# laurentsenta/testground

Measured on AMD Instinct MI355X. Metric: simulated packets/sec (whole node) at 10k & 1M peers; % of HBM roofline, higher is better.
Workload: dtype u32/u64 integer

## Files before the change

testground_amd/build.py:

```python
from __future__ import annotations

import os
import subprocess
from pathlib import Path

PKG = Path(__file__).resolve().parent
ROOT = PKG.parent
CSRC = PKG / "csrc"
LIB = PKG / "libtgsim.so"
SOURCES = [CSRC / "tgsim_kernels.hip", CSRC / "tgsim_engine.cpp", CSRC / "tgsim_bridge.cpp", CSRC / "tgsim_comm.cpp"]
HEADERS = [CSRC / "tgsim_internal.h", CSRC / "tgsim_launch.h", ROOT / "include" / "tgsim.h"]
ORACLE_DIR = ROOT / "oracle"
ORACLE_LIB = ORACLE_DIR / "build" / "libtgoracle.so"

HIPCC = os.environ.get("HIPCC", "/opt/rocm/bin/hipcc")
ARCH = os.environ.get("PYTORCH_ROCM_ARCH", "gfx950")


def _stale(target: Path, deps) -> bool:
    if not target.exists():
        return True
    t = target.stat().st_mtime
    return any(Path(d).stat().st_mtime > t for d in deps)


PROF_LIB = PKG / "libtgsim_prof.so"
CHECK_LIB = PKG / "libtgsim_check.so"


def build_engine(force: bool = False, verbose: bool = False, profile: bool = False, check: bool = False) -> Path:
    lib = PROF_LIB if profile else CHECK_LIB if check else LIB
    if not force and not _stale(lib, SOURCES + HEADERS):
        return lib
    objs = []
    build_dir = PKG / ("build_prof" if profile else "build_check" if check else "build")
    build_dir.mkdir(exist_ok=True)
    for src in SOURCES:
        obj = build_dir / (src.stem + ".o")
        dev = ["-mllvm", "-amdgpu-use-amdgpu-trackers=1", "-mllvm", "-disable-promote-alloca-to-lds"] \
            if src.suffix == ".hip" else []
        cmd = [HIPCC, f"--offload-arch={ARCH}", "-O3", "-std=c++17", "-fPIC", "-Wall", *dev,
               "-Wno-unused-result", *(["-DTGSIM_PROFILE"] if profile else []),
               *(["-DTGSIM_CHECK"] if check else []), "-c", str(src), "-o", str(obj)]
        if verbose:
            print(" ".join(cmd))
        subprocess.run(cmd, check=True)
        objs.append(str(obj))
    cmd = [HIPCC, f"--offload-arch={ARCH}", "-shared", "-fPIC", "-o", str(lib), *objs]
    if verbose:
        print(" ".join(cmd))
    subprocess.run(cmd, check=True)
    return lib


def build_oracle(force: bool = False) -> Path:
    if os.environ.get("TGORACLE_LIB"):
        return Path(os.environ["TGORACLE_LIB"])
    if force or _stale(ORACLE_LIB, [ORACLE_DIR / "tgoracle.c", ORACLE_DIR / "tgoracle.h", ROOT / "include" / "tgsim.h"]):
        subprocess.run(["make", "-C", str(ORACLE_DIR), "-B" if force else "all"], check=True,
                       stdout=subprocess.DEVNULL)
    return ORACLE_LIB


MOCK_DIR = ROOT / "tests" / "mockrccl"
# ... 37 lines not shown
```

testground_amd/csrc/tgsim_internal.h:

```cpp
#pragma once
#include <hip/hip_runtime.h>
#include <stdint.h>

#include "../../include/tgsim.h"

namespace tgsim {

constexpr uint32_t kHeapCap = 1024;
constexpr uint32_t kWave = 64;
#ifndef TGSIM_SPW
#define TGSIM_SPW 1
#endif
constexpr uint32_t kSpw = TGSIM_SPW;
constexpr uint32_t kAhead = kWave / kSpw;
constexpr uint64_t kEMask = (1ull << 46) - 1;
constexpr uint32_t kStates = TGSIM_SYNC_STATES;
constexpr uint32_t kDeadDst = 0xFFFFFFFFu;

struct alignas(16) SrcParams {
  uint64_t lat_ns;
  uint64_t burst_ns;
  int32_t sigma;
  uint32_t mult;
  uint32_t shift_ext;
// ... 49 lines not shown
  uint32_t last_dup, last_cor, last_reo, _pad;
  SrcParams p;
};

enum StatSlot {
  kStOffered = 0, kStScheduled, kStCloned, kStCorrupted, kStVerdict0,
  kStBytes = 12, kStErr = 13, kStQueue = 14, kStLost = 15, kStFlushed = 16,
  kStCarrySkip = 17,
  kStBktRecs = 18,
  kStSlots = 20
};
#ifndef TGSIM_STAT_COPIES
#define TGSIM_STAT_COPIES 2048
#endif
constexpr uint32_t kStatCopies = TGSIM_STAT_COPIES;
constexpr uint32_t kErrTimeOverflow = 1u;

struct SimArgs {
  const SrcParams* params;
  SrcState* state;
  const uint8_t* enabled;
  const uint32_t* ip;
  const Interval* rules;
  const uint64_t* off;
  const InRec* in;
  uint8_t* verdict;
  uint4* heap;
  uint64_t* ring;
  tgsim_delivery* emit;
  uint32_t* emit_n;
  unsigned long long* stats;
  uint32_t key0, key1;
  uint32_t n_src, shard_begin, n_peers, queue_limit;
  uint32_t any_disabled;
  uint64_t t0_ns, tick_ns, horizon_ns;
  const uint32_t* order;
  uint64_t* stamps;
  unsigned long long* dst_cnt;
  uint64_t* err_host;
  uint32_t* worklist;
  tgsim_delivery* emit_pool;
  uint32_t* emit_pool_idx;
  uint32_t* g_first;
  uint64_t* g_pend;
  const uint64_t* g_fwd;
  uint32_t g_floods, g_degree;
  tgsim_delivery* dst_bkt;
  uint32_t emit_r : 24, bkt_log : 7, dst_slot : 1;
  uint32_t emit_pool_cap;
  uint4* wheel;
  WheelMeta* wmeta;
};
static_assert(sizeof(SimArgs) == 280, "SimArgs layout");
constexpr uint32_t kStampSlots = 32;

constexpr uint32_t kFuseMax = 8;
struct FusedWindow {
  const uint64_t* off;
  const InRec* in;
  uint8_t* verdict;
  tgsim_delivery* emit;
  uint32_t* emit_n;
  unsigned long long* dst_cnt;
  uint64_t t0_ns, horizon_ns;
};
struct FusedArgs {
  FusedWindow w[kFuseMax];
  uint32_t n_win;
  uint32_t step_base;
  uint32_t ticket_base;
  uint32_t* ticket;
  uint32_t* done;
  uint32_t prio_n;
  uint32_t persistent;
};
constexpr uint32_t kErrHandoff = 2u;
constexpr uint32_t kErrDeliverCap = 4u;
constexpr uint32_t kErrEmitPool = 8u;

struct EmitRead {
  const tgsim_delivery* base;
  const tgsim_delivery* pool;
  const uint32_t* pool_idx;
  uint32_t r;
  uint32_t slot;
  const tgsim_delivery* bkt;
  uint32_t bkt_log, _pad;
  const uint64_t* guard_total;
  uint64_t guard_cap;
};
constexpr uint32_t kSlotShift = 46;
constexpr uint32_t kBktLogMin = 3, kBktLogMax = 6;
#if defined(TGSIM_CHECK) && !defined(TGSIM_CHECK_FULL_SLOTS)
constexpr uint64_t kSlotNone = (1u << kBktLogMax) + 3;
#else
constexpr uint64_t kSlotNone = (1ull << (64 - kSlotShift)) - 1;
#endif
static_assert(kSlotNone >= (1u << kBktLogMax), "the fallback places records behind every bucket slot");
__host__ __device__ inline uint64_t slot_bits(unsigned long long rank) {
  return (uint64_t)(rank < kSlotNone ? rank : kSlotNone) << kSlotShift;
}
__host__ __device__ inline const tgsim_delivery* emit_rec(const EmitRead& e, uint32_t s, uint64_t o0, uint64_t o1,
                                                         uint32_t i, uint32_t pidx) {
  const uint64_t cap = 2 * (o1 - o0) + e.r;
  return i < cap ? e.base + 2 * o0 + (uint64_t)e.r * s + i : e.pool + pidx + (i - cap);
}
struct GroupDeliver {
// ... 50 lines not shown
```

testground_amd/csrc/tgsim_kernels.hip:

```cpp
#include <errno.h>
#include <stdlib.h>
#include "tgsim_launch.h"

namespace tgsim {

__device__ __forceinline__ void philox(uint32_t c0, uint32_t c1, uint32_t c2, uint32_t c3,
                                       uint32_t k0, uint32_t k1, uint32_t r[4]) {
  __asm__ volatile("" : "+s"(k0), "+s"(k1));
#pragma unroll
  for (int i = 0; i < 10; ++i) {
    const uint64_t p0 = (uint64_t)0xD2511F53u * c0, p1 = (uint64_t)0xCD9E8D57u * c2;
    const uint32_t h0 = (uint32_t)(p0 >> 32), l0 = (uint32_t)p0;
    const uint32_t h1 = (uint32_t)(p1 >> 32), l1 = (uint32_t)p1;
    const uint32_t n0 = h1 ^ c1 ^ k0, n2 = h0 ^ c3 ^ k1;
    c0 = n0; c1 = l1; c2 = n2; c3 = l0;
    k0 += 0x9E3779B9u;
    k1 += 0xBB67AE85u;
  }
  r[0] = c0; r[1] = c1; r[2] = c2; r[3] = c3;
}

__device__ __forceinline__ uint32_t crand(uint32_t raw, uint32_t rho, uint32_t& last) {
  if (rho == 0) return raw;
  const uint64_t r = (uint64_t)rho + 1;
  const uint32_t a = (uint32_t)(((uint64_t)raw * ((1ull << 32) - r) + (uint64_t)last * r) >> 32);
  last = a;
  return a;
}

__device__ __forceinline__ uint64_t w0_of(const uint4& a) {
  return ((uint64_t)a.y << 32) | a.x;
}
__device__ __forceinline__ bool item_lt(const uint4& a, const uint4& b) {
  const uint64_t ea = w0_of(a) & kEMask, eb = w0_of(b) & kEMask;
  const bool dup_first = (a.y >> 30 & 1u) > (b.y >> 30 & 1u);
  const bool seq_lt = (a.z < b.z) | ((a.z == b.z) & dup_first);
  return (ea < eb) | ((ea == eb) & seq_lt);
}

template <uint32_t kCap>
struct SimLdsT {
  uint4 slot[kCap];
  uint32_t wcnt[kWheelB];
  uint32_t whdr[4];
};
static_assert(sizeof(SimLdsT<kHeapCap>) <= 65536, "simulate workgroup LDS");

constexpr uint32_t kFvPass = 0xFFu;

#ifdef TGSIM_CHECK
__device__ unsigned int tg_exec_faults;
__device__ unsigned int tg_exec_lines[8192];
__device__ __noinline__ void tg_exec_fault(const char* what, uint64_t exec, uint32_t l, int line) {
  const uint32_t me = __lane_id();
// ... 64 lines not shown
__device__ __forceinline__ void scan_maxplus(uint64_t& a, uint64_t& b, int line = __builtin_LINE()) {
#define STEP(C, R) { const uint64_t pa = dpp64<C, R>(0, a, line), pb = dpp64<C, R>(0, b, line); \
                     const uint64_t nb = pb + a; b = nb > b ? nb : b; a = pa + a; }
  TG_SCAN_STEPS(STEP)
#undef STEP
}
__device__ __forceinline__ int32_t scan_sum_i32(int32_t v, int line = __builtin_LINE()) {
#define STEP(C, R) v += (int32_t)dpp<C, R>(0u, (uint32_t)v, line);
  TG_SCAN_STEPS(STEP)
#undef STEP
  return v;
}
__device__ __forceinline__ int32_t scan_max_i32(int32_t v, int line = __builtin_LINE()) {
#define STEP(C, R) v = max(v, (int32_t)dpp<C, R>(0x80000000u, (uint32_t)v, line));
  TG_SCAN_STEPS(STEP)
#undef STEP
  return v;
}
__device__ __forceinline__ uint32_t scan_max_u32(uint32_t v, int line = __builtin_LINE()) {
#define STEP(C, R) v = max(v, dpp<C, R>(0u, v, line));
  TG_SCAN_STEPS(STEP)
#undef STEP
  return v;
}
__device__ __forceinline__ uint64_t scan_max_u64(uint64_t v, int line = __builtin_LINE()) {
#define STEP(C, R) { const uint64_t p = dpp64<C, R>(0ull, v, line); v = p > v ? p : v; }
  TG_SCAN_STEPS(STEP)
#undef STEP
  return v;
}
__device__ __forceinline__ uint64_t scan_min_u64(uint64_t v, int line = __builtin_LINE()) {
#define STEP(C, R) { const uint64_t p = dpp64<C, R>(~0ull, v, line); v = p < v ? p : v; }
  TG_SCAN_STEPS(STEP)
#undef STEP
  return v;
}

__device__ __forceinline__ uint32_t count_le_sorted_u32(uint32_t v, uint32_t t, int line = __builtin_LINE()) {
  TG_FULL_EXEC_AT("count_le_sorted", line);
  uint32_t lo = 0;
#pragma unroll
  for (uint32_t s = 32; s; s >>= 1)
    if ((uint32_t)__shfl(v, (int)(lo + s - 1), 64) <= t) lo += s;
  return lo + ((uint32_t)__shfl(v, (int)lo, 64) <= t ? 1u : 0u);
}

__device__ __forceinline__ uint64_t delayed(const SrcParams& p, uint64_t T, uint32_t raw) {
  if (p.sigma == 0) return T + p.lat_ns;
  const uint32_t m = 2u * (uint32_t)p.sigma;
  const int64_t delay = (int64_t)(raw % m) + (int64_t)p.lat_ns - (int64_t)p.sigma;
  return delay > 0 ? T + (uint64_t)delay : T;
}

struct RecvFold {
  uint32_t* first;
  uint64_t* pend;
  const uint64_t* fwd;
  uint32_t floods, degree, shard_begin, n_local;
  uint64_t tick_ns;
  double inv_tick;
};
__device__ __forceinline__ RecvFold recv_fold(const SimArgs& a) {
  return RecvFold{a.g_first, a.g_pend,  a.g_fwd,   a.g_floods,
                  a.g_degree, a.shard_begin, a.n_src, a.tick_ns, 1.0 / (double)a.tick_ns};
}
__device__ __forceinline__ void fold_receipt(const RecvFold& g, uint32_t dst, uint32_t seq, uint32_t flags, uint64_t d,
                                             uint64_t fw) {
  const uint32_t f = seq / g.degree, s = dst - g.shard_begin;
  if (s >= g.n_local || f >= g.floods || (flags & TGSIM_FLAG_CORRUPT) || (fw >> f & 1ull)) return;
  uint64_t q = (uint64_t)((double)d * g.inv_tick);
  const int64_t r = (int64_t)(d - q * g.tick_ns);
  q = r < 0 ? q - 1 : (uint64_t)r >= g.tick_ns ? q + 1 : q;
  uint64_t t = q + 1;
  if (t > 0xFFFFFFFEull) t = 0xFFFFFFFEull;
  if (__hip_atomic_fetch_min(&g.first[(uint64_t)s * 64 + f], (uint32_t)t, __ATOMIC_RELAXED, __HIP_MEMORY_SCOPE_AGENT) ==
      0xFFFFFFFFu)
    __hip_atomic_fetch_or(&g.pend[s], 1ull << f, __ATOMIC_RELAXED, __HIP_MEMORY_SCOPE_AGENT);
}

struct EmitOut {
  tgsim_delivery* region;
  tgsim_delivery* over;
  uint32_t cap;
  __device__ __forceinline__ bool fits(uint32_t i) const { return i < cap || over != nullptr; }
  __device__ __forceinline__ tgsim_delivery* at(uint32_t i) const { return i < cap ? region + i : over + (i - cap); }
};
__device__ __forceinline__ EmitOut emit_out(const SimArgs& a, uint32_t s, uint64_t sbeg, uint64_t send) {
  EmitOut o;
  o.region = a.emit + 2 * sbeg + (uint64_t)a.emit_r * s;
  o.over = nullptr;
  o.cap = (uint32_t)(2 * (send - sbeg)) + a.emit_r;
  return o;
}
__device__ __forceinline__ void emit_claim(const SimArgs& a, uint32_t s, EmitOut& o, uint32_t total, uint32_t lane) {
  if (total <= o.cap) return;
  const uint32_t need = total - o.cap;
  uint32_t at = 0;
  if (lane == 0) at = atomicAdd(a.worklist - 2, need);
  at = (uint32_t)__builtin_amdgcn_readfirstlane((int)at);
  if ((uint64_t)at + need <= a.emit_pool_cap) {
    o.over = a.emit_pool + at;
    if (lane == 0) a.emit_pool_idx[s] = at;
  } else if (lane == 0) {
    atomicOr(&a.stats[kStErr], (unsigned long long)kErrEmitPool);
    if (a.err_host) __hip_atomic_store(a.err_host, (uint64_t)kErrEmitPool, __ATOMIC_RELAXED, __HIP_MEMORY_SCOPE_SYSTEM);
  }
}

__device__ __forceinline__ uint32_t fib_lookup(const Interval* iv, uint32_t n, uint32_t ip) {
  uint32_t lo = 0, hi = n;
  while (lo < hi) {
    const uint32_t mid = (lo + hi) >> 1;
    if (iv[mid].hi < ip) lo = mid + 1;
    else hi = mid;
  }
  if (lo < n && iv[lo].lo <= ip) return iv[lo].act;
  return TGSIM_ACCEPT;
}

__device__ __forceinline__ uint32_t filter(const SimArgs& a, const SrcParams& p, bool src_on, uint32_t dst) {
  if (dst == TGSIM_EXTERNAL) {
    if (!src_on) return TGSIM_V_DISCONNECTED;
    return (p.shift_ext >> 8 & 1u) ? TGSIM_V_EXTERNAL : TGSIM_V_NO_ROUTE;
  }
  if (!src_on || (a.any_disabled && !a.enabled[dst])) return TGSIM_V_DISCONNECTED;
  if (p.rule_n) {
    const uint32_t act = fib_lookup(a.rules + p.rule_off, p.rule_n, a.ip[dst]);
    if (act == TGSIM_DROP) return TGSIM_V_BLACKHOLE;
    if (act == TGSIM_REJECT) return TGSIM_V_PROHIBIT;
  }
  return kFvPass;
}

__device__ __forceinline__ uint64_t wave_sum(uint64_t v, int line = __builtin_LINE()) {
  TG_FULL_EXEC_AT("wave_sum", line);
#pragma unroll
  for (int o = 32; o > 0; o >>= 1) {
    const uint32_t lo = __shfl_xor((uint32_t)v, o, 64);
    const uint32_t hi = __shfl_xor((uint32_t)(v >> 32), o, 64);
    v += ((uint64_t)hi << 32) | lo;
  }
  return v;
}

__device__ __forceinline__ void wave_lds_sync() {
  __builtin_amdgcn_s_waitcnt(0xC07F);
  __builtin_amdgcn_wave_barrier();
  __asm__ volatile("" ::: "memory");
}

__device__ __forceinline__ void stamp(const SimArgs& a, uint32_t wg, uint32_t lane, uint32_t k, uint64_t v) {
  if (a.stamps && lane == 0) a.stamps[(size_t)wg * kStampSlots + k] = v;
}

#ifdef TGSIM_PROFILE
#define PROF_T0(n) const uint64_t _pt##n = __builtin_amdgcn_s_memtime()
#define PROF_ADD(k, n) (pf[k] += __builtin_amdgcn_s_memtime() - _pt##n)
#define PROF_CNT(k, v) (pf[k] += (v))
#else
#define PROF_T0(n) do {} while (0)
#define PROF_ADD(k, n) do {} while (0)
#define PROF_CNT(k, v) do {} while (0)
#endif

template <uint32_t J>
__device__ __forceinline__ uint32_t xor_lane(uint32_t v) {
  TG_FULL_EXEC("xor_lane");
  uint32_t r;
  if constexpr (J == 1) r = dpp<0xB1, 0xF>(0u, v, __LINE__);
  else if constexpr (J == 2) r = dpp<0x4E, 0xF>(0u, v, __LINE__);
  else if constexpr (J < 32) r = (uint32_t)__builtin_amdgcn_ds_swizzle((int)v, (int)(0x1Fu | (J << 10)));
  else r = (uint32_t)__shfl_xor((int)v, 32, 64);
  __asm__ volatile("" : "+v"(r));
  return r;
}
template <uint32_t K, uint32_t J>
__device__ __forceinline__ void sort_stage(uint4& v, uint32_t& vf, uint32_t lane) {
  const uint4 pv = make_uint4(xor_lane<J>(v.x), xor_lane<J>(v.y), xor_lane<J>(v.z), xor_lane<J>(v.w));
  const uint32_t pf = xor_lane<J>(vf);
  const bool m_lt = vf < pf || (vf == pf && item_lt(v, pv));
  const bool keep_min = ((lane & J) == 0) == ((lane & K) == 0);
  if (keep_min != m_lt) {
    v = pv;
    vf = pf;
  }
  if constexpr (J > 1) sort_stage<K, J / 2>(v, vf, lane);
}
template <uint32_t K>
__device__ __forceinline__ void sort_merge(uint4& v, uint32_t& vf, uint32_t lane) {
  sort_stage<K, K / 2>(v, vf, lane);
  if constexpr (K < kWave) sort_merge<K * 2>(v, vf, lane);
}
__device__ __forceinline__ void wave_sort_items(uint4& v, bool has, uint32_t lane) {
  uint32_t vf = has ? 0u : 1u;
  sort_merge<2>(v, vf, lane);
}

template <uint32_t kCap, bool kOver = false>
struct SimQueue {
  static constexpr uint32_t kSlotMask = kCap - 1;
  SimLdsT<kCap>& lds;
  const SrcParams& p;
  uint32_t lane;
  uint32_t rh, rn, qn, pn;
  uint32_t fn;
  uint32_t pk;
  uint32_t rpush;
  uint64_t B;
  uint64_t H;
  uint64_t tat;
  tgsim_delivery* emit;
  tgsim_delivery* over;
  uint32_t cap;
  unsigned long long* dcnt;
  bool dslot;
  tgsim_delivery* bkt;
  uint32_t bkt_log;
  RecvFold rf;
  uint32_t n_emit, src;
  uint32_t sched, corrupted, lost;
  uint64_t bytes;
#ifdef TGSIM_PROFILE
  uint64_t pf[24];
#endif

  __device__ __forceinline__ uint4& slot(uint32_t k) { return lds.slot[(rh + k) & kSlotMask]; }
  __device__ __forceinline__ uint64_t ring_d(uint32_t k) {
    const uint2 v = *reinterpret_cast<const uint2*>(&lds.slot[(rh + k) & kSlotMask]);
    return ((uint64_t)v.y << 32) | v.x;
  }

#ifdef TGSIM_CHECK
  __device__ void check(int tag) {
    uint32_t bad = 0;
    uint64_t be = 0;
    for (uint32_t k = lane; k < qn; k += kWave) {
      const uint64_t e = w0_of(slot(rn + k)) & kEMask;
      if (e >= B) { bad |= 1; be = e; }
      if (k + 1 < qn && item_lt(slot(rn + k + 1), slot(rn + k))) bad |= 2;
    }
    for (uint32_t k = lane; k < pn; k += kWave) {
      const uint64_t e = w0_of(slot(rn + qn + k)) & kEMask;
      if (e < B || e >= H) { bad |= 4; be = e; }
    }
    for (uint32_t k = lane; k < fn; k += kWave) {
      const uint64_t e = w0_of(slot(rn + qn + pn + k)) & kEMask;
      if (e < H || e < B) { bad |= 8 | (k << 8); be = e; }
    }
    if (B > H && pn) bad |= 16;
    const uint64_t m = __ballot(bad != 0);
    if (m) {
      const uint32_t l = (uint32_t)__builtin_ctzll(m);
      const uint32_t bb = readlane32(bad, l);
      const uint64_t ee = readlane64(be, l);
      if (lane == 0)
        printf("CHECK tag %d src %u rn %u qn %u pn %u fn %u B %llu H %llu bad %x e %llu lanes %llx\n", tag, src, rn, qn,
               pn, fn, (unsigned long long)B, (unsigned long long)H, bb, (unsigned long long)ee, (unsigned long long)m);
    }
  }
#define QCHECK(t) Q.check(t)
#else
#define QCHECK(t) do {} while (0)
#endif

  __device__ __forceinline__ void htb_scan(bool in, uint64_t e, uint32_t len, uint64_t& d,
                                           uint64_t& tat_after) const {
    const uint64_t c = ((uint64_t)len * p.mult) >> (p.shift_ext & 0xFFu);
    uint64_t A = in ? c : 0, B = in ? (e > p.burst_ns ? e - p.burst_ns : 0) + c : 0;
    scan_maxplus(A, B);
    const uint64_t ta = tat + A;
    tat_after = ta > B ? ta : B;
    const uint64_t before = shr1_u64(tat_after, tat);
    d = e > before ? e : before;
  }

  __device__ __forceinline__ void commit(bool c, uint32_t n, const uint4& qi, uint64_t d, uint64_t tat_after) {
// ... 443 lines not shown
  uint32_t g = kWheelGMin;
  while (g < kWheelGMax && (span >> g) > kWheelB - 2) ++g;
  return g;
}
constexpr uint32_t kWheelRebuildKeep = 32;
constexpr uint32_t kWheelCooldown = 16;
static_assert(sizeof(StatePair) == sizeof(SrcState), "SrcState hand-off");

constexpr int kModePlain = 0, kModeHandoff = 1;
constexpr uint32_t kRingFirst = 16;
template <bool kOpen, uint32_t kCap, int kMode = kModePlain, bool kRecv = false, bool kList = false>
__device__ __forceinline__ uint32_t sim_source(const SimArgs& a, const uint32_t s, const uint32_t wg, SimLdsT<kCap>& lds,
                                               uint32_t* claim = nullptr, uint32_t claim_base = 0) {
  const uint32_t lane = threadIdx.x;
  constexpr uint32_t kSlotMask = kCap - 1;
  stamp(a, wg, lane, 0, __builtin_amdgcn_s_memrealtime());
  const SrcParams pp = a.params[s];
  constexpr bool kH = kMode == kModeHandoff, kBounded = kMode != kModePlain;
  constexpr int kPol = kH ? kSc1 : 0;
  SrcState st;
  if constexpr (kH) {
    const auto rs = region(a.state + s, sizeof(SrcState));
    st = __builtin_bit_cast(SrcState, (StatePair{ld16<kSc1>(rs, 0), ld16<kSc1>(rs, 16)}));
  } else {
    st = a.state[s];
  }
  const auto rm = region(a.wmeta + s, sizeof(WheelMeta));
  const auto rw = region(a.wheel + (size_t)s * kWheelB * kWheelCB, kWheelB * kWheelCB * 16u);
  constexpr uint32_t kOff = 0xFFFFFFF0u;
  uint32_t wcnt = ld2<kPol>(rm, a.wmeta ? 2u * lane : kOff);
  const uint4 whd = ld16<kPol>(rm, a.wmeta ? 2u * kWheelB : kOff);
  const uint64_t sbeg = a.off[s], send = a.off[s + 1];
  const bool src_on = a.enabled[a.shard_begin + s] != 0;
  SimQueue<kCap, kList> Q{lds, pp, lane};
  Q.rh = 0;
  Q.rn = r_len(st);
  Q.rpush = 0;
  Q.qn = q_near(st);
  Q.pn = q_len(st) - q_near(st);
  Q.fn = 0;
  Q.H = a.horizon_ns;
  Q.tat = st.tat;
  Q.src = a.shard_begin + s;
  Q.emit = a.emit + 2 * sbeg + (uint64_t)(kList ? a.emit_r : kHeapCap) * s;
  Q.n_emit = 0;
  Q.dcnt = a.dst_cnt;
  Q.dslot = kList && a.dst_slot;
  Q.bkt = kList ? a.dst_bkt : nullptr;
  Q.bkt_log = a.bkt_log;
  Q.rf = kRecv ? recv_fold(a) : RecvFold{};
  Q.sched = Q.corrupted = Q.lost = 0;
  Q.bytes = 0;
#ifdef TGSIM_PROFILE
  for (int k = 0; k < 24; ++k) Q.pf[k] = 0;
  uint64_t* pf = Q.pf;
#endif
  const uint32_t rh0 = r_head(st), rn0 = Q.rn;
  uint32_t rl = 0;
  uint64_t idx = sbeg + lane;
  const uint64_t last_in = send > sbeg ? send - 1 : sbeg;
  InRec rec = {}, rec2 = {};
  uint32_t wbase = 0, wctl = 0, wdue = 0, nd = 0;
  uint64_t wlast = 0;
  auto wheel_item = [&](uint32_t c, bool& in) -> uint4 {
    TG_FULL_EXEC("ds_bpermute");
    const uint32_t rot = (uint32_t)__shfl((int)wdue, (int)((wbase + lane) & (kWheelB - 1)), 64);
    const uint32_t wincl = (uint32_t)scan_sum_i32((int32_t)rot), wexcl = wincl - rot;
    const uint32_t k = c + lane;
    uint32_t lo = 0;
#pragma unroll
    for (uint32_t sb = kWave / 2; sb; sb >>= 1)
      if ((uint32_t)__shfl((int)wincl, (int)(lo + sb - 1), 64) <= k) lo += sb;
    const uint32_t j = lo & (kWheelB - 1);
    const uint32_t idx = k - (uint32_t)__shfl((int)wexcl, (int)j, 64);
    in = k < nd;
    return ld16<kPol>(rw, in ? 16u * (((wbase + j) & (kWheelB - 1)) * kWheelCB + idx) : kOff);
  };
  uint64_t moved = 0;
  {
    const uint64_t* gr = a.ring + (size_t)s * kHeapCap;
    const uint4* gh = a.heap + (size_t)s * kHeapCap;
    const uint32_t rn = Q.rn, qn = Q.qn + Q.pn;
    uint64_t rv0;
    uint4 qv[kCap / kWave];
    if constexpr (kBounded) {
      const auto rr = region(gr, 8u * kHeapCap), rq = region(gh, 16u * qn);
      rv0 = ld8<kPol>(rr, lane < kRingFirst ? 8u * ((rh0 + (lane < rn ? lane : 0u)) & (kHeapCap - 1)) : kOff);
#pragma unroll
      for (uint32_t u = 0; u < kCap / kWave; ++u) qv[u] = ld16<kPol>(rq, 16u * (u * kWave + lane));
    } else {
      const uint32_t ql = qn ? qn - 1 : 0, qh = q_head(st);
      rv0 = gr[(rh0 + (lane < rn && lane < kRingFirst ? lane : 0u)) & (kHeapCap - 1)];
#pragma unroll
      for (uint32_t u = 0; u < kCap / kWave; ++u) {
        const uint32_t k = u * kWave + lane;
        qv[u] = gh[(qh + (k < qn ? k : ql)) & (kHeapCap - 1)];
      }
    }
    if (send > sbeg) {
      rec = a.in[idx < send ? idx : last_in];
      rec2 = a.in[idx + kWave < send ? idx + kWave : last_in];
    }
    if (q_parked(st)) {
      wbase = (uint32_t)__builtin_amdgcn_readfirstlane((int)whd.x);
      wctl = (uint32_t)__builtin_amdgcn_readfirstlane((int)whd.y);
      const bool all = kList || (wctl >> 8 & 1u);
      wlast = (Q.H - 1) >> (wctl & 0xFFu);
// ... 18 lines not shown
      stop = __ballot(k < rn && v >= Q.H) != 0;
    }
    moved = 8ull * rl + 16ull * qn;
    const uint32_t nq = Q.qn;
    const uint64_t below = (1ull << lane) - 1;
    uint32_t cs = 0, cf = 0;
#pragma unroll
    for (uint32_t u = 0; u < kCap / kWave; ++u) {
      const uint32_t k = u * kWave + lane;
      const bool pool = k >= nq && k < qn;
      const bool soon = pool && (w0_of(qv[u]) & kEMask) < Q.H;
      const uint64_t msn = __ballot(soon), mfr = __ballot(pool && !soon);
      uint32_t d = k;
      if (soon) d = nq + cs + (uint32_t)__popcll(msn & below);
      else if (pool) d = qn - 1 - cf - (uint32_t)__popcll(mfr & below);
      if (k < qn) lds.slot[(rn + d) & kSlotMask] = qv[u];
      cs += (uint32_t)__popcll(msn);
      cf += (uint32_t)__popcll(mfr);
    }
    Q.pn = cs;
    Q.fn = cf;
    Q.append_pool(win0, wv0);
  }
  for (uint32_t c = kWave; c < nd; c += kWave) {
    bool in;
    const uint4 v = wheel_item(c, in);
    Q.append_pool(in, v);
  }
  Q.pk = readlane32((uint32_t)scan_sum_i32((int32_t)wcnt), kWave - 1);
  if (Q.pk && wlast > wbase) wbase = (uint32_t)wlast;
  if constexpr (kList) {
    EmitOut eo = emit_out(a, s, sbeg, send);
    emit_claim(a, s, eo, Q.qn + Q.pn + (uint32_t)(2 * (send - sbeg)), lane);
    Q.over = eo.over;
    Q.cap = eo.cap;
  }
  if (q_parked(st)) moved += sizeof(WheelMeta) + 16ull * nd;
  lds.wcnt[lane] = wcnt;
  if (lane == 0) {
    lds.whdr[0] = wbase;
    lds.whdr[1] = wctl;
    lds.whdr[2] = nd;
    lds.whdr[3] = rh0 + rn0;
  }
#ifndef TGSIM_PROFILE
  stamp(a, wg, lane, 11, rl | (uint64_t)rn0 << 16);
#endif
#ifndef TGSIM_PROFILE
  stamp(a, wg, lane, 10, __builtin_amdgcn_s_memrealtime());
#endif
  const bool plain = src_on && !a.any_disabled && pp.rule_n == 0;
  const uint32_t ext_v = (pp.shift_ext >> 8 & 1u) ? TGSIM_V_EXTERNAL : TGSIM_V_NO_ROUTE;
  const bool corr = (pp.rho_dup | pp.rho_cor | pp.rho_reo) != 0;
  const uint32_t lim = a.queue_limit;
  uint32_t last_dup = st.last_dup, last_cor = st.last_cor, last_reo = st.last_reo;
  unsigned long long* const sc = a.stats + (size_t)(wg % kStatCopies) * kStSlots;
  {
    const uint64_t b0 = 16ull * (Q.qn + Q.pn + Q.fn + Q.pk) + 8ull * Q.rn;
    if (lane == 0 && b0) atomicAdd(&sc[kStQueue], (unsigned long long)b0);
    if (lane == 0 && b0 != moved) atomicAdd(&sc[kStCarrySkip], (unsigned long long)(b0 - moved));
  }
  uint64_t vc_lo = 0, vc_hi = 0;
  uint32_t n_clone = 0;
  auto flush_verdicts = [&]() {
#pragma unroll
    for (uint32_t k = 0; k < 8; ++k) {
      const uint32_t f = (uint32_t)(((k < 4 ? vc_lo : vc_hi) >> (16u * (k & 3u))) & 0xFFFFu);
      const uint32_t tot = readlane32((uint32_t)scan_sum_i32((int32_t)f), kWave - 1);
      if (lane == 0 && tot) atomicAdd(&sc[kStVerdict0 + k], (unsigned long long)tot);
    }
    vc_lo = vc_hi = 0;
  };
  uint32_t perr = 0;
  wave_lds_sync();
  Q.B = Q.qn ? (w0_of(Q.slot(Q.rn + Q.qn - 1)) & kEMask) + 1 : a.t0_ns;
  QCHECK(1);
  stamp(a, wg, lane, 1, __builtin_amdgcn_s_memrealtime());

  const uint32_t n_batches = (uint32_t)((send - sbeg + kWave - 1) / kWave);
  const bool open_q = kOpen || (!corr && (uint64_t)Q.rn + Q.qn + Q.pn + Q.fn + Q.pk + 2 * (send - sbeg) < lim);
  uint64_t T_enq = 0;
  uint64_t v_idx = 0;
  uint32_t v_out = 0;
  bool v_pend = false;
  for (uint32_t b = 0; b < n_batches; ++b) {
    PROF_T0(b);
    const uint64_t my_idx = idx;
    const bool staged = my_idx < send;
    const InRec r = rec;
    idx += kWave;
    rec = rec2;
    rec2 = a.in[idx + kWave < send ? idx + kWave : last_in];
    if (v_pend) a.verdict[v_idx] = (uint8_t)v_out;
    const uint64_t T = a.t0_ns + (uint64_t)r.tick * a.tick_ns;
    const uint32_t len = r.len & 0xFFFFu;
    uint32_t fv = 0u;
    if (plain) fv = r.dst == TGSIM_EXTERNAL ? ext_v : kFvPass;
    else if (staged) fv = filter(a, pp, src_on, r.dst);
    if (!staged) fv = 0u;
    uint32_t vout = 0xF0u | fv;
    if (kOpen || !corr) {
      bool cand = false, reo_o = false;
      uint32_t cst = 0, flo = 0, flc = TGSIM_FLAG_DUP;
      uint64_t ec = ~0ull;
      if (staged && fv == kFvPass) {
        uint32_t r0[4];
        philox(Q.src, r.dst, r.seq, 0, a.key0, a.key1, r0);
        const int count = 1 + (pp.thr_dup && pp.thr_dup >= r0[0]) - (pp.thr_loss && pp.thr_loss >= r0[1]);
        if (count == 0) {
          vout = 0xF0u | TGSIM_V_LOSS;
        } else {
          cand = true;
          if (count == 2) {
            uint32_t r2[4];
            philox(Q.src, r.dst, r.seq, 2, a.key0, a.key1, r2);
            if (pp.thr_loss && pp.thr_loss >= r2[0]) {
              cst = 1;
            } else {
              cst = 2;
              if (pp.thr_cor && pp.thr_cor >= r2[1]) flc |= TGSIM_FLAG_CORRUPT;
              ec = (pp.thr_reo && pp.thr_reo >= r2[2]) ? T : delayed(pp, T, r2[3]);
              if (ec > kEMask) { perr = 1; ec = kEMask; }
            }
          }
          flo = (pp.thr_cor && pp.thr_cor >= r0[2]) ? TGSIM_FLAG_CORRUPT : 0u;
          reo_o = pp.thr_reo && pp.thr_reo >= r0[3];
        }
      }
      PROF_ADD(0, b);
      PROF_T0(w);
      if (open_q) {
        uint64_t eo = reo_o ? T : T + pp.lat_ns;
        const bool need1 = cand && !reo_o && pp.sigma != 0;
        if (__ballot(need1)) {
          if (need1) {
            uint32_t r1[4];
            philox(Q.src, r.dst, r.seq, 1, a.key0, a.key1, r1);
            eo = delayed(pp, T, r1[0]);
          }
        }
        if (cand && eo > kEMask) { perr = 1; eo = kEMask; }
        if (cand) {
          const uint32_t cv = cst == 0 ? TGSIM_V_NONE : cst == 1 ? TGSIM_V_LOSS : TGSIM_V_SCHEDULED;
          vout = (cv << 4) | TGSIM_V_SCHEDULED;
        }
        Q.insert(cand, make_item(eo, len, flo, r.seq, r.dst));
        Q.insert(cand && cst == 2, make_item(ec, len, flc, r.seq, r.dst));
        const uint64_t mc = __ballot(cand);
        if (mc) T_enq = readlane64(T, 63u - (uint32_t)__builtin_clzll(mc));
      }
      uint64_t pend = (kOpen || open_q) ? 0ull : __ballot(cand);
      if constexpr (!kOpen) while (pend) {
        PROF_CNT(3, 1);
        if (Q.rn + Q.qn + Q.pn + Q.fn + Q.pk >= lim) {
          const uint64_t qh = Q.qn ? (w0_of(Q.slot(Q.rn)) & kEMask) : Q.pn ? Q.B : (Q.fn | Q.pk) ? Q.H : ~0ull;
          const uint64_t dh = Q.rn ? Q.ring_d(0) : ~0ull;
          const uint64_t t_ev = qh < dh ? qh : dh;
          const uint64_t mf = __ballot(((pend >> lane) & 1ull) && T <= t_ev);
          if (mf) {
            if ((mf >> lane) & 1ull) {
              const uint32_t cv = cst == 0 ? TGSIM_V_NONE : cst == 1 ? TGSIM_V_LOSS : TGSIM_V_QUEUE_FULL;
              vout = (cv << 4) | TGSIM_V_QUEUE_FULL;
            }
            pend &= ~mf;
            PROF_CNT(2, 1);
            continue;
          }
        }
        const uint32_t w0 = (uint32_t)__builtin_ctzll(pend);
        const uint32_t wl = 63u - (uint32_t)__builtin_clzll(pend);
        const uint64_t T_last = readlane64(T, wl);
        QCHECK(10);
        Q.refill(T_last);
        QCHECK(8);
        PROF_T0(s1);
        const bool hq = lane < Q.qn;
        const uint4 qi = hq ? Q.slot(Q.rn + lane) : make_uint4(0, 0, 0, 0);
        const uint64_t qe = hq ? (w0_of(qi) & kEMask) : ~0ull;
        const bool inS = qe < T_last;
        const uint32_t nS = ballot_count(inS);
        uint64_t T_cut = ~0ull;
        if (nS == kWave && Q.qn > kWave) {
          const uint64_t e64 = w0_of(Q.slot(Q.rn + kWave)) & kEMask;
          if (e64 < T_last) T_cut = e64;
        }
        uint64_t dS = 0, tatS = 0;
        if (nS) Q.htb_scan(inS, qe, qi.y >> 14 & 0xFFFFu, dS, tatS);
        PROF_ADD(7, s1);
        PROF_T0(s2);
        const bool inw = cand && ((pend >> lane) & 1ull) && T <= T_cut;
        const uint64_t mw = __ballot(inw);
        uint32_t D = 0;
        const uint64_t T_mx = mw ? readlane64(T, 63u - (uint32_t)__builtin_clzll(mw)) : 0ull;
        if (mw) {
          const uint64_t T_max = T_mx;
          for (uint32_t base = 0;; base += kWave) {
            const uint32_t k = base + lane;
            const uint32_t ks = k - Q.rn;
            uint64_t dep = ~0ull;
            if (base + kWave > Q.rn && nS) {
              const uint64_t dfs = shfl64(dS, (k >= Q.rn && ks < kWave) ? ks : 0u);
              if (k >= Q.rn && ks < nS) dep = dfs;
            }
            if (k < Q.rn) dep = Q.ring_d(k);
            const uint64_t stop = __ballot(dep >= T_max);
            const uint32_t nd = stop ? (uint32_t)__builtin_ctzll(stop) : kWave;
            const bool carry = D == base;
            if (nd > 16) {
              const uint64_t pm = scan_max_u64(lane < nd ? dep : ~0ull);
              uint32_t lo = 0;
#pragma unroll
              for (uint32_t sb = 32; sb; sb >>= 1)
                if (shfl64(pm, lo + sb - 1) < T) lo += sb;
              lo += shfl64(pm, lo) < T ? 1u : 0u;
              if (carry) D += lo;
            } else {
              bool alive = carry;
              for (uint32_t l = 0; l < nd; ++l) {
                const uint64_t dl = readlane64(dep, l);
                alive = alive && dl < T;
                D += alive ? 1u : 0u;
              }
            }
            if (nd < kWave) break;
          }
        }
        PROF_ADD(8, s2);
        PROF_T0(s3);
        const uint32_t Dm = scan_max_u32(inw ? D : 0u);
        const int32_t delta = (int32_t)(Dm - shr1_u32(Dm, 0u));
        const int32_t cnt = inw ? 1 + (cst == 2) : 0;
        const int32_t P = scan_sum_i32(cnt - delta);
        const int32_t M = scan_max_i32(P);
        const int32_t x0 = (int32_t)(Q.rn + Q.qn + Q.pn + Q.fn + Q.pk), ilim = (int32_t)lim;
        const int32_t Pex = (int32_t)shr1_u32((uint32_t)P, 0u);
        const int32_t Mex = (int32_t)shr1_u32((uint32_t)M, 0u);
        const int32_t xb = Pex + min(x0, ilim - Mex);
        const int32_t y = xb - delta;
        const bool clone_adm = inw && cst == 2 && y < ilim;
        const bool orig_adm = inw && y + (cst == 2 ? 1 : 0) < ilim;
        uint64_t eo = reo_o ? T : T + pp.lat_ns;
        const bool need1 = orig_adm && !reo_o && pp.sigma != 0;
        if (__ballot(need1)) {
          if (need1) {
            uint32_t r1[4];
            philox(Q.src, r.dst, r.seq, 1, a.key0, a.key1, r1);
            eo = delayed(pp, T, r1[0]);
          }
        }
        if (orig_adm && eo > kEMask) { perr = 1; eo = kEMask; }
        PROF_ADD(9, s3);
        PROF_T0(s4);
        uint64_t ea = clone_adm ? ec : ~0ull;
        if (orig_adm && eo < ea) ea = eo;
        const uint64_t madm = __ballot((orig_adm || clone_adm) && ea < T_mx);
        uint32_t wend = kWave;
        if (madm) {
          uint64_t beta = ~0ull;
          for (uint64_t mm = madm; mm; mm &= mm - 1) {
            const uint32_t i = (uint32_t)__builtin_ctzll(mm);
            const uint64_t ei = readlane64(ea, i);
            const uint32_t pe = ballot_count(inS && qe < ei);
            const uint64_t b1 = pe < nS ? readlane64(dS, pe) : ~0ull;
            const uint64_t tb = pe == 0 ? Q.tat : readlane64(tatS, pe - 1);
            const uint64_t b2 = ei > tb ? ei : tb;
            if (lane == i) beta = b1 < b2 ? b1 : b2;
          }
          const uint64_t Bex = shr1_u64(scan_min_u64(beta), ~0ull);
          const uint64_t mv = __ballot(inw && Bex < T);
          if (mv) wend = (uint32_t)__builtin_ctzll(mv);
          PROF_CNT(23, mv ? 1u : 0u);
        }
        const bool inwin = inw && lane < wend;
        const uint64_t mwin = __ballot(inwin);
        uint64_t T_w, e_new = ~0ull;
        uint32_t Dw = 0, lw = 0;
        if (mwin) {
          lw = 63u - (uint32_t)__builtin_clzll(mwin);
          T_w = readlane64(T, lw);
          Dw = readlane32(D, lw);
          if (madm) e_new = readlane64(scan_min_u64(inwin ? ea : ~0ull), kWave - 1);
        } else {
          T_w = readlane64(T, w0);
        }
        PROF_ADD(10, s4);
        PROF_T0(s5);
        const uint64_t t_c = e_new < T_w ? e_new : T_w;
        const bool inC = inS && qe < t_c;
        const uint32_t nC = ballot_count(inC);
        if (nC) Q.commit(inC, nC, qi, dS, tatS);
        QCHECK(5);
        Q.rh = (Q.rh + Dw) & kSlotMask;
        Q.rn -= Dw;
        PROF_ADD(11, s5);
        if (inwin) {
          const uint32_t cv = cst == 0 ? TGSIM_V_NONE
                            : cst == 1 ? TGSIM_V_LOSS
                                       : (clone_adm ? TGSIM_V_SCHEDULED : TGSIM_V_QUEUE_FULL);
          vout = (cv << 4) | (orig_adm ? TGSIM_V_SCHEDULED : TGSIM_V_QUEUE_FULL);
        }
        Q.insert(inwin && orig_adm, make_item(eo, len, flo, r.seq, r.dst));
        QCHECK(6);
        Q.insert(inwin && clone_adm, make_item(ec, len, flc, r.seq, r.dst));
        QCHECK(7);
        if (e_new < T_w) {
          PROF_T0(s6);
          Q.serve_until(T_w);
          PROF_ADD(12, s6);
          QCHECK(9);
        }
        if (mwin) pend &= lw >= 63u ? 0ull : ~((1ull << (lw + 1)) - 1);
        QCHECK(2);
      }
      PROF_ADD(1, w);
    } else if constexpr (!kOpen) {
      uint4 r0 = make_uint4(0, 0, 0, 0), r2 = make_uint4(0, 0, 0, 0);
      uint32_t r1x = 0;
      if (staged && fv == kFvPass) {
        uint32_t t[4];
        philox(Q.src, r.dst, r.seq, 0, a.key0, a.key1, t);
        r0 = make_uint4(t[0], t[1], t[2], t[3]);
        if (pp.thr_dup) {
          philox(Q.src, r.dst, r.seq, 2, a.key0, a.key1, t);
          r2 = make_uint4(t[0], t[1], t[2], t[3]);
        }
        if (pp.sigma) {
          philox(Q.src, r.dst, r.seq, 1, a.key0, a.key1, t);
          r1x = t[0];
        }
      }
      const uint32_t n_st = ballot_count(staged);
      for (uint32_t j = 0; j < n_st; ++j) {
        if (readlane32(fv, j) != kFvPass) continue;
        const uint64_t Tj = readlane64(T, j);
        const uint32_t dj = readlane32(r.dst, j), sj = readlane32(r.seq, j), lj = readlane32(len, j);
        const uint4 a0 = make_uint4(readlane32(r0.x, j), readlane32(r0.y, j), readlane32(r0.z, j), readlane32(r0.w, j));
        int count = 1;
        if (pp.thr_dup && pp.thr_dup >= crand(a0.x, pp.rho_dup, last_dup)) ++count;
        if (pp.thr_loss && pp.thr_loss >= a0.y) --count;
        uint32_t vj;
        if (count == 0) {
          vj = 0xF0u | TGSIM_V_LOSS;
        } else {
          auto enq = [&](uint32_t reo_raw, uint32_t delay_raw, uint32_t fl) -> uint32_t {
            Q.serve_until(Tj);
            Q.depart_before(Tj);
            if (Q.rn + Q.qn + Q.pn + Q.fn + Q.pk >= lim) return TGSIM_V_QUEUE_FULL;
            bool reordered = false;
            if (pp.thr_reo) reordered = !(pp.thr_reo < crand(reo_raw, pp.rho_reo, last_reo));
            uint64_t e = reordered ? Tj : delayed(pp, Tj, delay_raw);
            if (e > kEMask) { perr = 1; e = kEMask; }
            Q.insert(lane == 0, make_item(e, lj, fl, sj, dj));
            return TGSIM_V_SCHEDULED;
          };
          uint32_t cv = TGSIM_V_NONE;
          if (count == 2) {
            const uint4 a2 = make_uint4(readlane32(r2.x, j), readlane32(r2.y, j), readlane32(r2.z, j), readlane32(r2.w, j));
            if (pp.thr_loss && pp.thr_loss >= a2.x) {
              cv = TGSIM_V_LOSS;
            } else {
              uint32_t fl = TGSIM_FLAG_DUP;
              if (pp.thr_cor && pp.thr_cor >= crand(a2.y, pp.rho_cor, last_cor)) fl |= TGSIM_FLAG_CORRUPT;
              cv = enq(a2.z, a2.w, fl);
            }
          }
          uint32_t fl = 0;
          if (pp.thr_cor && pp.thr_cor >= crand(a0.z, pp.rho_cor, last_cor)) fl |= TGSIM_FLAG_CORRUPT;
          const uint32_t ov = enq(a0.w, readlane32(r1x, j), fl);
          vj = (cv << 4) | ov;
        }
        if (lane == j) vout = vj;
      }
    }
    v_pend = staged;
    v_idx = my_idx;
    v_out = vout;
    if (staged) {
      const uint32_t vo = vout & 15u, vc = vout >> 4;
      const uint64_t uo = 1ull << (16u * (vo & 3u)), uc = 1ull << (16u * (vc & 3u));
      if (vo < 4) vc_lo += uo;
      else vc_hi += uo;
      if (vc < 4) vc_lo += uc;
      else if (vc < 8) vc_hi += uc;
      n_clone += vc != TGSIM_V_NONE ? 1u : 0u;
    }
    if ((b & 0x3FFFu) == 0x3FFFu) flush_verdicts();
  }
  if (v_pend) a.verdict[v_idx] = (uint8_t)v_out;
  stamp(a, wg, lane, 2, __builtin_amdgcn_s_memrealtime());
  if (open_q && T_enq) {
    Q.serve_until(T_enq);
    Q.depart_before(T_enq);
  }
  QCHECK(3);
  PROF_T0(e);
  Q.serve_until(a.horizon_ns);
  QCHECK(4);
  PROF_ADD(13, e);
  if (lane == 0) a.emit_n[s] = Q.n_emit;
  stamp(a, wg, lane, 3, __builtin_amdgcn_s_memrealtime());
  uint32_t next_ticket = 0;
  if (claim && lane == 0) next_ticket = atomicAdd(claim, 1u) - claim_base;
  uint32_t pk_end = Q.pk;
  uint64_t moved_end = 0;
  if constexpr (!kList) {
    const uint32_t fn0 = a.wheel ? Q.fn : 0u;
    const auto rm = region(a.wmeta + s, sizeof(WheelMeta));
    const auto rw = region(a.wheel + (size_t)s * kWheelB * kWheelCB, kWheelB * kWheelCB * 16u);
    wbase = lds.whdr[0];
    wctl = lds.whdr[1];
    nd = lds.whdr[2];
    wcnt = lds.wcnt[lane];
    if (fn0) {
      const uint32_t f0 = Q.rn + Q.qn + Q.pn;
      if (!Q.pk) {
        wctl = (wctl & 0xFFFF0000u) | wheel_width(pp.lat_ns + (uint64_t)(pp.sigma > 0 ? pp.sigma : 0));
        lds.wcnt[lane] = 0;
        wave_lds_sync();
      }
      const uint32_t g0 = wctl & 0xFFu;
      uint64_t mn = ~0ull;
      for (uint32_t k = lane; k < fn0; k += kWave) {
        const uint64_t e = w0_of(Q.slot(f0 + k)) & kEMask;
        mn = e < mn ? e : mn;
      }
      mn >>= g0;
// ... 40 lines not shown
      st2<kPol>(rm, 2u * lane, wcnt);
      if (lane == 0) st16<kPol>(rm, 2u * kWheelB, make_uint4(wbase, wctl, 0u, 0u));
      moved_end += sizeof(WheelMeta);
    }
  }
  {
    uint64_t* gr = a.ring + (size_t)s * kHeapCap;
    uint4* gh = a.heap + (size_t)s * kHeapCap;
    const uint32_t r_new = Q.rpush < Q.rn ? Q.rpush : Q.rn;
    const uint32_t rh1 = (lds.whdr[3] + Q.rpush - Q.rn) & (kHeapCap - 1);
    moved_end += 8ull * r_new + 16ull * (Q.qn + Q.pn + Q.fn);
    if constexpr (kH) {
      const auto rr = region(gr, kHeapCap * 8u), rq = region(gh, kHeapCap * 16u);
      for (uint32_t k = Q.rn - r_new + lane; k < Q.rn; k += kWave)
        st8<kSc1>(rr, 8u * ((rh1 + k) & (kHeapCap - 1)), Q.ring_d(k));
      for (uint32_t k = lane; k < Q.qn + Q.pn + Q.fn; k += kWave) st16<kSc1>(rq, 16u * k, Q.slot(Q.rn + k));
    } else {
      for (uint32_t k = Q.rn - r_new + lane; k < Q.rn; k += kWave) gr[(rh1 + k) & (kHeapCap - 1)] = Q.ring_d(k);
      for (uint32_t k = lane; k < Q.qn + Q.pn + Q.fn; k += kWave) gh[k] = Q.slot(Q.rn + k);
    }
    uint32_t near_out = Q.qn;
    if constexpr (kList) {
      const uint32_t tot = Q.qn + Q.pn + Q.fn;
      if (Q.pn + Q.fn) {
        bool bad = false;
        for (uint32_t k = lane + 1; k < tot; k += kWave) bad |= item_lt(Q.slot(Q.rn + k), Q.slot(Q.rn + k - 1));
        if (__ballot(bad) == 0) near_out = tot;
      }
    }
    if (lane == 0) {
      SrcState ns;
      ns.tat = Q.tat;
      ns.heap_n = q_pack(Q.qn + Q.pn + Q.fn, pk_end);
      ns.near_n = near_out;
      ns.ring_n = r_pack(Q.rn, rh1);
      ns.last_dup = last_dup;
      ns.last_cor = last_cor;
      ns.last_reo = last_reo;
      if constexpr (kH) {
        const auto rs = region(a.state + s, sizeof(SrcState));
        const StatePair sp = __builtin_bit_cast(StatePair, ns);
        st16<kSc1>(rs, 0, sp.lo);
        st16<kSc1>(rs, 16, sp.hi);
      } else {
        a.state[s] = ns;
      }
    }
  }
  stamp(a, wg, lane, 4, __builtin_amdgcn_s_memrealtime());
  stamp(a, wg, lane, 5, ((uint64_t)s << 32) | n_batches);
  stamp(a, wg, lane, 6, __builtin_amdgcn_s_getreg((4 << 0) | (0 << 6) | (31 << 11)));
  stamp(a, wg, lane, 7, ((uint64_t)(Q.qn + Q.pn + Q.fn) << 32) | Q.rn);
#ifdef TGSIM_PROFILE
  for (int k = 0; k < 24; ++k) stamp(a, wg, lane, 8 + k, Q.pf[k]);
#endif
  const uint32_t sched = readlane32((uint32_t)scan_sum_i32((int32_t)Q.sched), kWave - 1);
  const uint32_t corrupted = readlane32((uint32_t)scan_sum_i32((int32_t)Q.corrupted), kWave - 1);
  const uint32_t lost = readlane32((uint32_t)scan_sum_i32((int32_t)Q.lost), kWave - 1);
  const uint64_t bytes = wave_sum(Q.bytes);
  const uint64_t qbytes = 16ull * (Q.qn + Q.pn + Q.fn + pk_end) + 8ull * Q.rn;
  const bool err = __ballot(perr != 0) != 0;
  const uint32_t c_clone = readlane32((uint32_t)scan_sum_i32((int32_t)n_clone), kWave - 1);
  flush_verdicts();
  if (lane == 0) {
    if (send > sbeg) atomicAdd(&sc[kStOffered], (unsigned long long)(send - sbeg));
    if (sched) atomicAdd(&sc[kStScheduled], (unsigned long long)sched);
    if (kList && a.dst_bkt && sched > Q.n_emit) atomicAdd(&sc[kStBktRecs], (unsigned long long)(sched - Q.n_emit));
    if (c_clone) atomicAdd(&sc[kStCloned], (unsigned long long)c_clone);
    if (corrupted) atomicAdd(&sc[kStCorrupted], (unsigned long long)corrupted);
    if (lost) atomicAdd(&sc[kStLost], (unsigned long long)lost);
    if (bytes) atomicAdd(&sc[kStBytes], (unsigned long long)bytes);
    if (qbytes) atomicAdd(&sc[kStQueue], (unsigned long long)qbytes);
    if (qbytes != moved_end) atomicAdd(&sc[kStCarrySkip], (unsigned long long)(qbytes - moved_end));
    if (err) {
      atomicOr(&a.stats[kStErr], (unsigned long long)kErrTimeOverflow);
      if (a.err_host)
        __hip_atomic_store(a.err_host, (uint64_t)kErrTimeOverflow, __ATOMIC_RELAXED, __HIP_MEMORY_SCOPE_SYSTEM);
    }
  }
  return (uint32_t)__builtin_amdgcn_readfirstlane((int)next_ticket);
}

__global__ __launch_bounds__(kWave, 3) void k_sim(SimArgs a) {
  __shared__ SimLdsT<kHeapCap> lds;
  const uint32_t s = a.order ? a.order[blockIdx.x] : blockIdx.x;
  if (s >= a.n_src) return;
  sim_source<false, kHeapCap>(a, s, blockIdx.x, lds);
}

__global__ __launch_bounds__(kWave, 3) void k_sim_recv(SimArgs a) {
  __shared__ SimLdsT<kHeapCap> lds;
  const uint32_t s = a.order ? a.order[blockIdx.x] : blockIdx.x;
  if (s >= a.n_src) return;
  sim_source<false, kHeapCap, kModePlain, true>(a, s, blockIdx.x, lds);
}

struct FusedSim {
  SimArgs w[kFuseMax];
};
__device__ __forceinline__ const SimArgs& kernarg_window(uint32_t k) {
  using KernargSimArgs = __attribute__((address_space(4))) const SimArgs;
  const KernargSimArgs* ka =
      (KernargSimArgs*)((__attribute__((address_space(4))) const char*)__builtin_amdgcn_kernarg_segment_ptr() +
                        k * sizeof(SimArgs));
  return *(const SimArgs*)ka;
}

// ... 2147 lines not shown
```

Baseline: 38.30 billion.

## Use reciprocal fastmod for jitter delay and cache per-record delay draw across retries

Adds a reciprocal-multiply modulo helper, computed once per source, and uses it in place of the 32-bit integer modulo when computing jittered delays. In the admission retry loop, the philox draw and delay computation for the original copy are now cached per lane, so they are no longer recomputed on every pass while a record stays pending. Profiling slots are widened and new counters added for these paths. The fastmod's correction step only subtracts the modulus once, which relies on the quotient estimate being off by at most one. The cached value must stay valid across retries of the same record.

```diff
diff --git a/testground_amd/build.py b/testground_amd/build.py
--- a/testground_amd/build.py
+++ b/testground_amd/build.py
@@ -9,7 +9,7 @@
 CSRC = PKG / "csrc"
 LIB = PKG / "libtgsim.so"
 SOURCES = [CSRC / "tgsim_kernels.hip", CSRC / "tgsim_engine.cpp", CSRC / "tgsim_bridge.cpp", CSRC / "tgsim_comm.cpp"]
-HEADERS = [CSRC / "tgsim_internal.h", CSRC / "tgsim_launch.h", ROOT / "include" / "tgsim.h"]
+HEADERS = [CSRC / "tgsim_internal.h", CSRC / "tgsim_launch.h", CSRC / "tgsim_fastmod.h", ROOT / "include" / "tgsim.h"]
 ORACLE_DIR = ROOT / "oracle"
 ORACLE_LIB = ORACLE_DIR / "build" / "libtgoracle.so"
 
diff --git a/testground_amd/csrc/tgsim_fastmod.h b/testground_amd/csrc/tgsim_fastmod.h
--- /dev/null
+++ b/testground_amd/csrc/tgsim_fastmod.h
@@ -0,0 +1,20 @@
+#pragma once
+#include <stdint.h>
+
+#if defined(__HIPCC__) || defined(__CUDACC__)
+#define TGSIM_HD __host__ __device__
+#else
+#define TGSIM_HD
+#endif
+
+namespace tgsim {
+
+TGSIM_HD inline uint32_t fastmod_rcp(uint32_t m) { return m ? 0xFFFFFFFFu / m : 0u; }
+
+TGSIM_HD inline uint32_t fastmod_u32(uint32_t raw, uint32_t m, uint32_t rcp) {
+  const uint32_t q = (uint32_t)(((uint64_t)raw * rcp) >> 32);
+  const uint32_t r = raw - q * m;
+  return r >= m ? r - m : r;
+}
+
+}
diff --git a/testground_amd/csrc/tgsim_internal.h b/testground_amd/csrc/tgsim_internal.h
--- a/testground_amd/csrc/tgsim_internal.h
+++ b/testground_amd/csrc/tgsim_internal.h
@@ -125,7 +125,8 @@
   WheelMeta* wmeta;
 };
 static_assert(sizeof(SimArgs) == 280, "SimArgs layout");
-constexpr uint32_t kStampSlots = 32;
+constexpr uint32_t kProfSlots = 32;
+constexpr uint32_t kStampSlots = 8 + kProfSlots;
 
 constexpr uint32_t kFuseMax = 8;
 struct FusedWindow {
diff --git a/testground_amd/csrc/tgsim_kernels.hip b/testground_amd/csrc/tgsim_kernels.hip
--- a/testground_amd/csrc/tgsim_kernels.hip
+++ b/testground_amd/csrc/tgsim_kernels.hip
@@ -1,5 +1,6 @@
 #include <errno.h>
 #include <stdlib.h>
+#include "tgsim_fastmod.h"
 #include "tgsim_launch.h"
 
 namespace tgsim {
@@ -170,6 +171,12 @@
   return delay > 0 ? T + (uint64_t)delay : T;
 }
 
+__device__ __forceinline__ uint64_t delayed(const SrcParams& p, uint64_t T, uint32_t raw, uint32_t rcp) {
+  if (p.sigma == 0) return T + p.lat_ns;
+  const int64_t delay = (int64_t)fastmod_u32(raw, 2u * (uint32_t)p.sigma, rcp) + (int64_t)p.lat_ns - (int64_t)p.sigma;
+  return delay > 0 ? T + (uint64_t)delay : T;
+}
+
 struct RecvFold {
   uint32_t* first;
   uint64_t* pend;
@@ -275,10 +282,16 @@
 #define PROF_T0(n) const uint64_t _pt##n = __builtin_amdgcn_s_memtime()
 #define PROF_ADD(k, n) (pf[k] += __builtin_amdgcn_s_memtime() - _pt##n)
 #define PROF_CNT(k, v) (pf[k] += (v))
+#define PROF_TAIL_VAR() uint64_t _pt_tail = 0
+#define PROF_TAIL_T0() (_pt_tail = __builtin_amdgcn_s_memtime())
+#define PROF_TAIL_ADD(k) (pf[k] += _pt_tail ? __builtin_amdgcn_s_memtime() - _pt_tail : 0)
 #else
 #define PROF_T0(n) do {} while (0)
 #define PROF_ADD(k, n) do {} while (0)
 #define PROF_CNT(k, v) do {} while (0)
+#define PROF_TAIL_VAR() do {} while (0)
+#define PROF_TAIL_T0() do {} while (0)
+#define PROF_TAIL_ADD(k) do {} while (0)
 #endif
 
 template <uint32_t J>
@@ -339,7 +352,7 @@
   uint32_t sched, corrupted, lost;
   uint64_t bytes;
 #ifdef TGSIM_PROFILE
-  uint64_t pf[24];
+  uint64_t pf[kProfSlots];
 #endif
 
   __device__ __forceinline__ uint4& slot(uint32_t k) { return lds.slot[(rh + k) & kSlotMask]; }
@@ -889,7 +902,7 @@
   Q.sched = Q.corrupted = Q.lost = 0;
   Q.bytes = 0;
 #ifdef TGSIM_PROFILE
-  for (int k = 0; k < 24; ++k) Q.pf[k] = 0;
+  for (int k = 0; k < (int)kProfSlots; ++k) Q.pf[k] = 0;
   uint64_t* pf = Q.pf;
 #endif
   const uint32_t rh0 = r_head(st), rn0 = Q.rn;
@@ -1014,6 +1027,7 @@
   const bool plain = src_on && !a.any_disabled && pp.rule_n == 0;
   const uint32_t ext_v = (pp.shift_ext >> 8 & 1u) ? TGSIM_V_EXTERNAL : TGSIM_V_NO_ROUTE;
   const bool corr = (pp.rho_dup | pp.rho_cor | pp.rho_reo) != 0;
+  const uint32_t sig_rcp = fastmod_rcp(2u * (uint32_t)pp.sigma);
   const uint32_t lim = a.queue_limit;
   uint32_t last_dup = st.last_dup, last_cor = st.last_cor, last_reo = st.last_reo;
   unsigned long long* const sc = a.stats + (size_t)(wg % kStatCopies) * kStSlots;
@@ -1045,7 +1059,9 @@
   uint64_t v_idx = 0;
   uint32_t v_out = 0;
   bool v_pend = false;
+  PROF_TAIL_VAR();
   for (uint32_t b = 0; b < n_batches; ++b) {
+    PROF_TAIL_ADD(24);
     PROF_T0(b);
     const uint64_t my_idx = idx;
     const bool staged = my_idx < send;
@@ -1081,7 +1097,7 @@
             } else {
               cst = 2;
               if (pp.thr_cor && pp.thr_cor >= r2[1]) flc |= TGSIM_FLAG_CORRUPT;
-              ec = (pp.thr_reo && pp.thr_reo >= r2[2]) ? T : delayed(pp, T, r2[3]);
+              ec = (pp.thr_reo && pp.thr_reo >= r2[2]) ? T : delayed(pp, T, r2[3], sig_rcp);
               if (ec > kEMask) { perr = 1; ec = kEMask; }
             }
           }
@@ -1112,6 +1128,8 @@
         if (mc) T_enq = readlane64(T, 63u - (uint32_t)__builtin_clzll(mc));
       }
       uint64_t pend = (kOpen || open_q) ? 0ull : __ballot(cand);
+      constexpr uint64_t kNoDraw = ~0ull;
+      uint64_t eo_drawn = kNoDraw;
       if constexpr (!kOpen) while (pend) {
         PROF_CNT(3, 1);
         if (Q.rn + Q.qn + Q.pn + Q.fn + Q.pk >= lim) {
@@ -1203,13 +1221,16 @@
         const bool orig_adm = inw && y + (cst == 2 ? 1 : 0) < ilim;
         uint64_t eo = reo_o ? T : T + pp.lat_ns;
         const bool need1 = orig_adm && !reo_o && pp.sigma != 0;
-        if (__ballot(need1)) {
-          if (need1) {
+        const bool draw1 = need1 && eo_drawn == kNoDraw;
+        if (__ballot(draw1)) {
+          PROF_CNT(25, (uint32_t)__popcll(__ballot(draw1)));
+          if (draw1) {
             uint32_t r1[4];
             philox(Q.src, r.dst, r.seq, 1, a.key0, a.key1, r1);
-            eo = delayed(pp, T, r1[0]);
+            eo_drawn = delayed(pp, T, r1[0], sig_rcp);
           }
         }
+        if (need1) eo = eo_drawn;
         if (orig_adm && eo > kEMask) { perr = 1; eo = kEMask; }
         PROF_ADD(9, s3);
         PROF_T0(s4);
@@ -1235,6 +1256,7 @@
         }
         const bool inwin = inw && lane < wend;
         const uint64_t mwin = __ballot(inwin);
+        PROF_CNT(26, (uint32_t)__popcll(__ballot(inwin && need1)));
         uint64_t T_w, e_new = ~0ull;
         uint32_t Dw = 0, lw = 0;
         if (mwin) {
@@ -1334,6 +1356,7 @@
         if (lane == j) vout = vj;
       }
     }
+    PROF_TAIL_T0();
     v_pend = staged;
     v_idx = my_idx;
     v_out = vout;
@@ -1480,7 +1503,7 @@
   stamp(a, wg, lane, 6, __builtin_amdgcn_s_getreg((4 << 0) | (0 << 6) | (31 << 11)));
   stamp(a, wg, lane, 7, ((uint64_t)(Q.qn + Q.pn + Q.fn) << 32) | Q.rn);
 #ifdef TGSIM_PROFILE
-  for (int k = 0; k < 24; ++k) stamp(a, wg, lane, 8 + k, Q.pf[k]);
+  for (int k = 0; k < (int)kProfSlots; ++k) stamp(a, wg, lane, 8 + k, Q.pf[k]);
 #endif
   const uint32_t sched = readlane32((uint32_t)scan_sum_i32((int32_t)Q.sched), kWave - 1);
   const uint32_t corrupted = readlane32((uint32_t)scan_sum_i32((int32_t)Q.corrupted), kWave - 1);
```

Result: faster. 39.39 billion (median of 6 runs) (+2.8%).
